# samuel-vitorino/lm.rs

Measured on AMD Instinct MI355X. Metric: decode tok/s + %HBM-roofline, Llama-3.2-1B Q8_0 @1/2/4/8 MI355X vs CPU ref, higher is better.
Workload: dtype int8xint8->int32, f32 combine; 1 GPU; llama-3.2-1b Q8_0 (gs=128) greedy decode, 5-token synthetic prompt then 3164 tokens, batch 1; parallelism=single GPU, image_bytes=1274634496

## Files before the change

lm.rs_amd/csrc/lmrs_kernels.hip:

```cpp
#include <hip/hip_ext.h>
#include <mutex>
#include <map>
#include <set>
#include <tuple>
#include <utility>

#include "lmrs_device_math.h"
#include "lmrs_kernels.h"
#include "lmrs_stage.h"

namespace lmrs {

constexpr int kBlock = 256;


constexpr int kMaxP = 16;

template <int NP>
__device__ __forceinline__ void rmsnorm_inplace(float4 (&v)[NP], const float4 (&wv)[NP], int n, float eps,
                                                int add_unit, float* scratch) {
    const int t = threadIdx.x;
    const int P = (n + 1023) >> 10;
    const int JP = (n >> 3) + 4;
#pragma unroll
// ... 49 lines not shown
            if (e < n) {
                float4 o;
                if (add_unit) {
                    o.x = (1.0f + wv[i].x) * (ss * v[i].x); o.y = (1.0f + wv[i].y) * (ss * v[i].y);
                    o.z = (1.0f + wv[i].z) * (ss * v[i].z); o.w = (1.0f + wv[i].w) * (ss * v[i].w);
                } else {
                    o.x = wv[i].x * (ss * v[i].x); o.y = wv[i].y * (ss * v[i].y);
                    o.z = wv[i].z * (ss * v[i].z); o.w = wv[i].w * (ss * v[i].w);
                }
                v[i] = o;
            }
        }
    }
}

template <bool Q4, int NP>
__device__ __forceinline__ void quantize_to_lds(const float4 (&v)[NP], int n, int8_t* xq, float* xs, void* gq, float* gs_out) {
    const int t = threadIdx.x;
    const int P = (n + 1023) >> 10;
#pragma unroll
    for (int i = 0; i < NP; ++i) {
        if (i < P) {
            const int e = i * 1024 + t * 4;
            const bool live = e < n;
            float m = 0.0f;
            if (live) m = fmaxf(fmaxf(fabsf(v[i].x), fabsf(v[i].y)), fmaxf(fabsf(v[i].z), fabsf(v[i].w)));
            m = group32_max(m);
            if (live) {
                if constexpr (!Q4) {
                    const float scale = m / 127.0f, inv = __builtin_amdgcn_rcpf(scale);
                    float dev = 0.0f;
                    int q0 = quant_q8_try(v[i].x, inv, dev), q1 = quant_q8_try(v[i].y, inv, dev);
                    int q2 = quant_q8_try(v[i].z, inv, dev), q3 = quant_q8_try(v[i].w, inv, dev);
                    if (quant_slow(m, dev)) { q0 = quant_q8(v[i].x, scale); q1 = quant_q8(v[i].y, scale); q2 = quant_q8(v[i].z, scale); q3 = quant_q8(v[i].w, scale); }
                    const unsigned packed = (q0 & 0xff) | ((q1 & 0xff) << 8) | ((q2 & 0xff) << 16) | ((unsigned)(q3 & 0xff) << 24);
                    *reinterpret_cast<unsigned*>(xq + e) = packed;
                    if ((t & 31) == 0) xs[e >> 7] = scale;
                    if (gq) {
                        *reinterpret_cast<unsigned*>(reinterpret_cast<int8_t*>(gq) + e) = packed;
                        if ((t & 31) == 0) gs_out[e >> 7] = scale;
                    }
                } else {
                    const float scale = m / -8.0f;
                    const unsigned a = quant_q4(v[i].x, scale), b = quant_q4(v[i].y, scale);
                    const unsigned c = quant_q4(v[i].z, scale), d = quant_q4(v[i].w, scale);
                    const int base = e & ~7, k0 = e & 7;
                    xq[base + (k0 >> 1) + 0] = (int8_t)((int)a - 8);
                    xq[base + 4 + (k0 >> 1) + 0] = (int8_t)((int)b - 8);
                    xq[base + (k0 >> 1) + 1] = (int8_t)((int)c - 8);
                    xq[base + 4 + (k0 >> 1) + 1] = (int8_t)((int)d - 8);
                    if ((t & 31) == 0) xs[e >> 7] = scale;
                    if (gq) {
                        uint8_t* g8 = reinterpret_cast<uint8_t*>(gq);
                        g8[(e >> 1) + 0] = (uint8_t)(a | (b << 4));
                        g8[(e >> 1) + 1] = (uint8_t)(c | (d << 4));
                        if ((t & 31) == 0) gs_out[e >> 7] = scale;
                    }
                }
            }
        }
    }
}

template <int NP>
__device__ __forceinline__ void load_vec(float4 (&v)[NP], const float* __restrict__ x, int n) {
    const int t = threadIdx.x;
    const int P = (n + 1023) >> 10;
#pragma unroll
    for (int i = 0; i < NP; ++i) {
        if (i < P) {
            const int e = i * 1024 + t * 4;
            if (e < n) v[i] = *reinterpret_cast<const float4*>(x + e);
        }
    }
}

struct TailPre { int pos, prompt_end; uint32_t tok_next; };
__device__ __forceinline__ TailPre tail_preload(const ArgmaxArgs& a) {
    TailPre p; p.pos = a.st->pos; p.prompt_end = a.st->prompt_end; p.tok_next = a.tokens[p.pos + 1]; return p;
}
__device__ __forceinline__ void argmax_tail(const ArgmaxArgs& a, float best, int best_i, int nan0, const TailPre& pre) {
    __shared__ float sv[kBlock / 64];
    __shared__ int si[kBlock / 64];
    __shared__ uint32_t s_next;
    if (threadIdx.x == 0 && a.tail_row > 0 && (0.0f > best || (0.0f == best && a.tail_row < best_i))) { best = 0.0f; best_i = a.tail_row; }
#pragma unroll
    for (int off = 32; off >= 1; off >>= 1) {
        const float ov = __shfl_xor(best, off); const int oi = __shfl_xor(best_i, off);
        if (ov > best || (ov == best && oi < best_i)) { best = ov; best_i = oi; }
    }
    if ((threadIdx.x & 63) == 0) { sv[threadIdx.x >> 6] = best; si[threadIdx.x >> 6] = best_i; }
    nan0 = __syncthreads_or(nan0);
    if (threadIdx.x == 0) {
        for (int w = 1; w < kBlock / 64; ++w)
            if (sv[w] > best || (sv[w] == best && si[w] < best_i)) { best = sv[w]; best_i = si[w]; }
        int win = best_i;
        if (nan0 || win == 0x7fffffff) win = 0;
        const int pos = pre.pos;
        uint32_t next = (uint32_t)win;
        if (pos + 1 >= pre.prompt_end) a.tokens[pos + 1] = next;
        else next = pre.tok_next;
        a.st->pos = pos + 1;
        a.st->step_count += 1;
        if (a.seq) *a.seq += 1u;
        s_next = next;
    }
    __syncthreads();
    const uint32_t token = s_next;
    if (a.emb.q4 == 0 && a.emb.dim > 0 && (a.emb.dim & 7) == 0 && a.emb.dim <= 8 * 4 * kBlock) {
        const int8_t* qrow = reinterpret_cast<const int8_t*>(a.emb.emb_q) + (size_t)token * a.emb.dim;
        const float* srow = a.emb.emb_s + ((size_t)token * a.emb.dim) / kGS;
        uint2 q8[4]; float sc[4];
#pragma unroll
        for (int k = 0; k < 4; ++k) {
            const int e = (k * kBlock + (int)threadIdx.x) * 8;
            const bool live = e < a.emb.dim;
            q8[k] = *reinterpret_cast<const uint2*>(qrow + (live ? e : 0));
            sc[k] = srow[(live ? e : 0) / kGS];
        }
#pragma unroll
        for (int k = 0; k < 4; ++k) {
            const int e = (k * kBlock + (int)threadIdx.x) * 8;
            if (e < a.emb.dim) {
                float o[8];
#pragma unroll
                for (int u = 0; u < 8; ++u) {
                    const int b = (int)(int8_t)(((u < 4 ? q8[k].x : q8[k].y) >> (8 * (u & 3))) & 0xff);
                    float v = (float)b * sc[k];
                    if (a.emb.do_scale) v = v * a.emb.scale;
                    o[u] = v;
                }
                *reinterpret_cast<float4*>(a.emb.x + e) = make_float4(o[0], o[1], o[2], o[3]);
                *reinterpret_cast<float4*>(a.emb.x + e + 4) = make_float4(o[4], o[5], o[6], o[7]);
            }
        }
    } else if (a.emb.q4 == 1 && a.emb.dim > 0 && (a.emb.dim & 7) == 0 && a.emb.dim <= 8 * 4 * kBlock) {
        const uint8_t* qrow = reinterpret_cast<const uint8_t*>(a.emb.emb_q) + ((size_t)token * a.emb.dim) / 2;
        const float* srow = a.emb.emb_s + ((size_t)token * a.emb.dim) / kGS;
        unsigned q4w[4]; float sc[4];
#pragma unroll
        for (int k = 0; k < 4; ++k) {
            const int e = (k * kBlock + (int)threadIdx.x) * 8;
            const bool live = e < a.emb.dim;
            q4w[k] = *reinterpret_cast<const unsigned*>(qrow + (live ? e : 0) / 2);
            sc[k] = srow[(live ? e : 0) / kGS];
        }
#pragma unroll
        for (int k = 0; k < 4; ++k) {
            const int e = (k * kBlock + (int)threadIdx.x) * 8;
            if (e < a.emb.dim) {
                float o[8];
#pragma unroll
                for (int u = 0; u < 8; ++u) {
                    const int nib = (int)((q4w[k] >> (4 * u)) & 0xfu) - 8;
                    float v = (float)nib * sc[k];
                    if (a.emb.do_scale) v = v * a.emb.scale;
                    o[u] = v;
                }
                *reinterpret_cast<float4*>(a.emb.x + e) = make_float4(o[0], o[1], o[2], o[3]);
                *reinterpret_cast<float4*>(a.emb.x + e + 4) = make_float4(o[4], o[5], o[6], o[7]);
            }
        }
    } else {
        for (int i = threadIdx.x; i < a.emb.dim; i += kBlock) {
            float v = dequant_elem(a.emb.emb_q, a.emb.emb_s, a.emb.q4, (size_t)token * a.emb.dim + i);
            if (a.emb.do_scale) v = v * a.emb.scale;
            a.emb.x[i] = v;
        }
    }
}

__device__ __forceinline__ unsigned cls_tag(const GemvArgs& a) { return (*a.tail.cls_seq + 1u) & 0x7ffu; }
__device__ __forceinline__ void cls_publish(const GemvArgs& a, int bid, unsigned tag, float best, int best_i) {
    const unsigned hi = best_i < 0 ? (0x80000000u | (tag << 20)) : ((tag << 20) | (best_i == 0x7fffffff ? 0xfffffu : (unsigned)best_i));
    __hip_atomic_store(a.tail.part_pk + bid, ((unsigned long long)hi << 32) | __float_as_uint(best), __ATOMIC_RELAXED, __HIP_MEMORY_SCOPE_AGENT);
}
__device__ __forceinline__ void cls_consumer(const GemvArgs& a, int nprod, const TailPre& pre, unsigned tag) {
    if (a.dbg && threadIdx.x == 0) a.dbg[4] = wall_clock64();
    float bv; int bi, nan0;
    for (unsigned spins = 0;; ++spins) {
        bv = __uint_as_float(0xff800000u); bi = 0x7fffffff; nan0 = 0;
        int ok = 1;
        for (int i = threadIdx.x; i < nprod; i += kBlock) {
            const unsigned long long pk = __hip_atomic_load(a.tail.part_pk + i, __ATOMIC_RELAXED, __HIP_MEMORY_SCOPE_AGENT);
            const unsigned hi = (unsigned)(pk >> 32);
            if (((hi >> 20) & 0x7ffu) != tag) { ok = 0; continue; }
            if (hi & 0x80000000u) { nan0 = 1; continue; }
            const float v = __uint_as_float((unsigned)pk); const int idx = (hi & 0xfffffu) == 0xfffffu ? 0x7fffffff : (int)(hi & 0xfffffu);
            if (v > bv || (v == bv && idx < bi)) { bv = v; bi = idx; }
        }
        if (__syncthreads_and(ok)) break;
// ... 701 lines not shown
                const int i = i0 + u;
                if constexpr (kBlock % HS4 == 0) { row[u] = r0 + i * (kBlock / HS4); col[u] = c4; }
                else { const int f = (int)threadIdx.x + i * kBlock; row[u] = f / HS4; col[u] = f - row[u] * HS4; }
                if constexpr (SCALE) sc[u] = rowscale[row[u] < nrows ? row[u] : nrows - 1];
            }
#pragma unroll
            for (int u = 0; u < 4; ++u) {
                const int i = i0 + u;
                if (i < NF && (AttGeom<HS>::ALIGNED || row[u] < nrows)) {
                    float4 v = rg[i];
                    if constexpr (SCALE) { v.x = sc[u] * v.x; v.y = sc[u] * v.y; v.z = sc[u] * v.z; v.w = sc[u] * v.w; }
                    *reinterpret_cast<float4*>(tile + row[u] * RS + col[u] * 4) = v;
                }
            }
        }
    }
    if (patch_t >= t0 && patch_t < t0 + ct) {
        const int fb = (patch_t - t0) * HS4, d = ((int)threadIdx.x - fb) & (kBlock - 1);
        if (d < HS4) {
            float4 v = *reinterpret_cast<const float4*>(patch + d * 4);
            if constexpr (SCALE) { const float ap = rowscale[patch_t - t0]; v.x = ap * v.x; v.y = ap * v.y; v.z = ap * v.z; v.w = ap * v.w; }
            *reinterpret_cast<float4*>(tile + (patch_t - t0) * RS + d * 4) = v;
        }
    }
}

#define ATT_STAMP(k) do { if (a.dbg && threadIdx.x == 0 && blockIdx.x == 0) a.dbg[k] = wall_clock64(); } while (0)

struct AttPre { float q0, q1, k0, k1; float2 cs; };

typedef float f32x4v __attribute__((ext_vector_type(4)));
__device__ __forceinline__ float* att_k_head(const AttnArgs& a, int kvh, int hs) {
    return a.k_cache + ((size_t)a.layer * a.n_kv_heads + kvh) * hs * (size_t)a.seq_len;
}
template <int NG>
__device__ __forceinline__ void att_kload(f32x4v (&dst)[NG], __amdgpu_buffer_rsrc_t krs, int voff, int g0, int S) {
#pragma unroll
    for (int u = 0; u < NG; ++u) {
        const auto t = __builtin_amdgcn_raw_buffer_load_b128(krs, voff, (g0 + u) * S * 16, 0);
        dst[u] = f32x4v{__uint_as_float(t[0]), __uint_as_float(t[1]), __uint_as_float(t[2]), __uint_as_float(t[3])};
    }
}
template <int NG>
__device__ __forceinline__ float att_kuse(float score, const f32x4v (&src)[NG], const float4* q4, int g0) {
#pragma unroll
    for (int u = 0; u < NG; ++u) {
        const float4 qq = q4[g0 + u];
        float pr;
        pr = qq.x * src[u].x; score = score + pr;
        pr = qq.y * src[u].y; score = score + pr;
        pr = qq.z * src[u].z; score = score + pr;
        pr = qq.w * src[u].w; score = score + pr;
    }
    return score;
}
template <int HS, int NG>
__device__ __forceinline__ float att_score_chain(f32x4v (&kk)[NG], __amdgpu_buffer_rsrc_t krs, int voff, const float* q, int S) {
    constexpr int HS4 = HS / 4;
    f32x4v kb[NG];
    float score = 0.0f;
    const float4* q4 = reinterpret_cast<const float4*>(q);
#pragma unroll
    for (int g0 = 0; g0 < HS4; g0 += 2 * NG) {
        if (g0 + NG < HS4) att_kload<NG>(kb, krs, voff, g0 + NG, S);
        score = att_kuse<NG>(score, kk, q4, g0);
        asm volatile("" : "+v"(score) : : "memory");
        if (g0 + NG < HS4) {
            if (g0 + 2 * NG < HS4) att_kload<NG>(kk, krs, voff, g0 + 2 * NG, S);
            score = att_kuse<NG>(score, kb, q4, g0 + NG);
            asm volatile("" : "+v"(score) : : "memory");
        }
    }
    return score;
}

__device__ __forceinline__ float2 rope_rotate(float v0, float v1, float fcr, float fci) {
    const float a0 = v0 * fcr, a1 = v1 * fci, b0 = v0 * fci, b1 = v1 * fcr;
    return make_float2(a0 - a1, b0 + b1);
}
__device__ __forceinline__ void k_store_pair(float* k, int S, int pos, int j, int half, float r0, float r1) {
    k[(((size_t)(j >> 2) * S + pos) << 2) + (j & 3)] = r0;
    k[(((size_t)((j + half) >> 2) * S + pos) << 2) + ((j + half) & 3)] = r1;
}
__device__ __forceinline__ float gemma_cap_window(float score, int wpos, int t) {
    score = score / 50.0f;
    score = (float)tanh((double)score);
    score = score * 50.0f;
    return score + (((unsigned)(wpos - t) <= 4096u) ? 0.0f : -2.3819763e38f);
}
template <int HS4>
__device__ __forceinline__ float tile_score(const float4* k, int ks, const float* qs) {
    constexpr int GB = 4;
    static_assert(HS4 % (2 * GB) == 0, "head size");
    const float4* q4 = reinterpret_cast<const float4*>(qs);
    auto dot = [](float score, const float4 (&q)[GB], const float4 (&kk)[GB]) __attribute__((always_inline)) {
#pragma unroll
        for (int u = 0; u < GB; ++u) {
            float pr;
            pr = q[u].x * kk[u].x; score = score + pr;
            pr = q[u].y * kk[u].y; score = score + pr;
            pr = q[u].z * kk[u].z; score = score + pr;
            pr = q[u].w * kk[u].w; score = score + pr;
        }
        return score;
    };
    float score = 0.0f;
    float4 ka[GB], qa[GB], kb[GB], qb[GB];
#pragma unroll
    for (int u = 0; u < GB; ++u) { ka[u] = k[u * ks]; qa[u] = q4[u]; }
#pragma unroll
    for (int g0 = 0; g0 < HS4; g0 += 2 * GB) {
#pragma unroll
        for (int u = 0; u < GB; ++u) { kb[u] = k[(g0 + GB + u) * ks]; qb[u] = q4[g0 + GB + u]; }
        asm volatile("" : "+v"(score) : : "memory");
        score = dot(score, qa, ka);
        if (g0 + 2 * GB < HS4) {
#pragma unroll
            for (int u = 0; u < GB; ++u) { ka[u] = k[(g0 + 2 * GB + u) * ks]; qa[u] = q4[g0 + 2 * GB + u]; }
        }
        asm volatile("" : "+v"(score) : : "memory");
        score = dot(score, qb, kb);
    }
    return score;
}
struct AttTag { const unsigned long long* gran; unsigned tag; int att_dim, kv_dim; int* err; };
template <int NG>
__device__ __forceinline__ void poll_granules(const unsigned long long* const (&gp)[NG], const AttTag& tg, int layer, unsigned long long (&xg)[NG]) {
    auto sweep = [&](unsigned long long (&x)[NG]) __attribute__((always_inline)) {
#pragma unroll
        for (int k = 0; k < NG; ++k) x[k] = __hip_atomic_load(gp[k], __ATOMIC_RELAXED, __HIP_MEMORY_SCOPE_AGENT);
    };
    auto fresh = [&](const unsigned long long (&x)[NG]) __attribute__((always_inline)) {
        bool ok = true;
#pragma unroll
        for (int k = 0; k < NG; ++k) ok = ok && (unsigned)(x[k] >> 32) == tg.tag;
        return __all(ok) != 0;
    };
    auto take = [&](const unsigned long long (&x)[NG]) __attribute__((always_inline)) {
#pragma unroll
        for (int k = 0; k < NG; ++k) xg[k] = x[k];
    };
    unsigned long long xa[NG], xb[NG];
    sweep(xa);
    for (unsigned spins = 0;; ++spins) {
        sweep(xb);
        if (fresh(xa)) { take(xa); break; }
        sweep(xa);
        if (fresh(xb)) { take(xb); break; }
        if (spins > kTagSpinMax || (spins & 1023) == 1023) {
            const int e = __hip_atomic_load(tg.err, __ATOMIC_RELAXED, __HIP_MEMORY_SCOPE_AGENT);
            if (e != 0 || spins > kTagSpinMax) {
                if (e == 0) __hip_atomic_store(tg.err, layer + 1, __ATOMIC_RELAXED, __HIP_MEMORY_SCOPE_AGENT);
                take(xb);
                break;
            }
        }
    }
}
__device__ __forceinline__ void granules_of(const AttTag& tg, int h, int kvh, int hs, int d, const unsigned long long** gp) {
    gp[0] = tg.gran + h * hs + d; gp[1] = tg.gran + tg.att_dim + kvh * hs + d; gp[2] = tg.gran + tg.att_dim + tg.kv_dim + kvh * hs + d;
}

template <int HS, int NF, bool COH, bool PRE = false, bool GEMMA = false, bool ROT = false, bool TAG = false>
__device__ __forceinline__ void attention_body(const AttnArgs& a, int h, int pos, char* smem, uint64_t etab, const AttPre& pre = AttPre(), const AttTag& tg = AttTag()) {
    static_assert(!PRE || HS / 2 <= kBlock, "one RoPE pair per lane");
    static_assert(!TAG || (HS <= kBlock && !COH && !PRE && !ROT), "granule polling: one value of each vector per lane");
// ... 259 lines not shown
        }
    }
    if (a.dbg && lane == 0 && blockIdx.x == 0) a.dbg[3] = wall_clock64();

    int wpos = pos;
    if constexpr (GEMMA) { const int wb = a.st->win_base; wpos = wb >= 0 ? wb : pos; }
    const float sqrt_hs = sqrtf((float)HS), ninf = __uint_as_float(0xff800000u);
    float sc[NPASS];
    float lmax = ninf;
#pragma unroll
    for (int p = 0; p < NPASS; ++p) {
        sc[p] = ninf;
        if (64 * p < T) {
            const int t = 64 * p + lane;
            float score = tile_score<HS4>(kt + t, TW, qs) / sqrt_hs;
            if constexpr (GEMMA) score = gemma_cap_window(score, wpos, t);
            sc[p] = t < T ? score : ninf;
            lmax = fmaxf(lmax, sc[p]);
        }
    }
    if (a.dbg && lane == 0 && blockIdx.x == 0) a.dbg[4] = wall_clock64();
    const float mx = wave64_max(lmax);
    float ex[NPASS];
#pragma unroll
    for (int p = 0; p < NPASS; ++p) {
        ex[p] = 0.0f;
        if (64 * p < T) {
            const int t = 64 * p + lane;
            const float e = expf_glibc_t(t < T ? sc[p] - mx : 0.0f, etab);
            ex[p] = t < T ? e : 0.0f;
        }
    }
    float sum = 0.0f;
#pragma unroll
    for (int p = 0; p < NPASS; ++p) {
        if (64 * p < T) {
            const int left = T - 64 * p;
            sum = wave_serial_sum(sum, ex[p], left >= 64 ? 4 : (left + 15) >> 4);
        }
    }
    float ap_lane = 0.0f;
#pragma unroll
    for (int p = 0; p < NPASS; ++p) {
        if (64 * p < T) {
            const int t = 64 * p + lane;
            const float w = ex[p] / sum;
            att[t] = t < pos ? w : 0.0f;
            if ((pos >> 6) == p) ap_lane = w;
        }
    }
    const float a_pos = __builtin_bit_cast(float, __builtin_amdgcn_readlane(__builtin_bit_cast(int, ap_lane), pos & 63));
    if (a.dbg && lane == 0 && blockIdx.x == 0) a.dbg[5] = wall_clock64();
    float o[ND];
#pragma unroll
    for (int i = 0; i < ND; ++i) o[i] = 0.0f;
#pragma unroll
    for (int t0 = 0; t0 < TW; t0 += 16) {
        if (t0 < pos) {
            float4 w4[4];
#pragma unroll
            for (int u = 0; u < 4; ++u) w4[u] = reinterpret_cast<const float4*>(att)[t0 / 4 + u];
#pragma unroll
            for (int u = 0; u < 4; ++u)
#pragma unroll
                for (int i = 0; i < ND; ++i) {
                    float pr;
                    pr = w4[u].x * v[i][t0 + 4 * u + 0]; o[i] = o[i] + pr;
                    pr = w4[u].y * v[i][t0 + 4 * u + 1]; o[i] = o[i] + pr;
                    pr = w4[u].z * v[i][t0 + 4 * u + 2]; o[i] = o[i] + pr;
                    pr = w4[u].w * v[i][t0 + 4 * u + 3]; o[i] = o[i] + pr;
                }
        }
    }
#pragma unroll
    for (int i = 0; i < ND; ++i) {
        const int d = lane + 64 * i;
        const float pr = a_pos * vnew[i];
        o[i] = o[i] + pr;
        if (d < HS) a.out[h * HS + d] = o[i];
    }
    if (a.dbg && lane == 0 && blockIdx.x == 0) a.dbg[7] = wall_clock64();
}

constexpr size_t kPairSmem = (size_t)(2 * 2 * 64 + 128 + 16 + 16) * 4 + (size_t)16 * 128 * 16 + (size_t)64 * 64 * 4;
template <bool GEMMA>
__device__ __forceinline__ void attention_pair_tag(const AttnArgs& a, const int h, const int pos, char* smem, const uint64_t etab, const AttTag& tg) {
    constexpr int HS = 64, HS4 = 16, TW = 128, half = 32;
    const int lane = threadIdx.x & 63, wv = __builtin_amdgcn_readfirstlane((int)threadIdx.x >> 6);
    const bool two = pos >= 64;
    if (wv > (two ? 1 : 0)) return;
    const int tb = two ? 64 * wv : 0;
    const int kv_mul = a.n_heads / a.n_kv_heads, kvh = h / kv_mul, kv_dim = a.n_kv_heads * HS;
    const int T = pos + 1, S = a.seq_len;
    float* base = reinterpret_cast<float*>(smem);
    float* qs = base + wv * 2 * HS;
    float* kn = qs + HS;
    float* att = base + 4 * HS;
    float* red = att + TW + 16;
    float4* kt = reinterpret_cast<float4*>(red + 16);
    float* prod = reinterpret_cast<float*>(kt + HS4 * TW);
    float* kT = att_k_head(a, kvh, HS);
    const float* vbase = a.v_cache + (size_t)a.layer * S * kv_dim + kvh * HS;
    if (a.dbg && lane == 0 && wv == 0 && blockIdx.x == 0) a.dbg[0] = wall_clock64();

    const float2 cs = *reinterpret_cast<const float2*>(a.rope + ((size_t)pos * half + (lane < half ? lane : 0)) * 2);
    if (tb < pos) {
#pragma unroll
        for (int g = 0; g < HS4; ++g)
            __builtin_amdgcn_global_load_lds((const LMRS_GLOBAL void*)(kT + ((size_t)g * S + tb + lane) * 4),
                                             (__attribute__((address_space(3))) void*)(kt + g * TW + tb), 16, 0, 0);
    }
    float v[64];
    const __amdgpu_buffer_rsrc_t vrs = __builtin_amdgcn_make_buffer_rsrc(const_cast<float*>(vbase), 0, 0x7fffffff, 0x00020000);
    const int vrow = kv_dim * 4, vb0 = tb * vrow;
    auto vblock = [&](auto self, auto u0c) __attribute__((always_inline)) -> void {
        constexpr int u0 = decltype(u0c)::value;
        if constexpr (u0 < 64) {
            if (tb + u0 < pos) {
#pragma unroll
                for (int u = 0; u < 16; ++u) v[u0 + u] = __uint_as_float(__builtin_amdgcn_raw_buffer_load_b32(vrs, lane * 4, vb0 + (u0 + u) * vrow, 0));
                self(self, std::integral_constant<int, u0 + 16>());
            }
        }
    };
    vblock(vblock, std::integral_constant<int, 0>());
#pragma unroll
    for (int u = 0; u < 64; ++u) { v[u] = tb + u < pos ? v[u] : 0.0f; asm volatile("" : "+v"(v[u])); }
    if (a.dbg && lane == 0 && wv == 0 && blockIdx.x == 0) a.dbg[1] = wall_clock64();

    unsigned long long xg[3];
    {
        const unsigned long long* gp[3];
        granules_of(tg, h, kvh, HS, lane, gp);
        poll_granules<3>(gp, tg, a.layer, xg);
    }
    asm volatile("s_waitcnt vmcnt(0)" ::: "memory");
    if (a.dbg && lane == 0 && wv == 0 && blockIdx.x == 0) a.dbg[2] = wall_clock64();
    const float vnew = __uint_as_float((unsigned)xg[2]);
    qs[lane] = __uint_as_float((unsigned)xg[0]); kn[lane] = __uint_as_float((unsigned)xg[1]);
    if (lane < half) {
        const int j = lane;
        const float2 rq = rope_rotate(qs[j], qs[j + half], cs.x, cs.y);
        qs[j] = rq.x; qs[j + half] = rq.y;
        const float2 rk = rope_rotate(kn[j], kn[j + half], cs.x, cs.y);
        if (wv == 0) k_store_pair(kT, S, pos, j, half, rk.x, rk.y);
        if ((pos >> 6) == (two ? wv : 0)) k_store_pair(reinterpret_cast<float*>(kt), TW, pos, j, half, rk.x, rk.y);
    }
    if (a.dbg && lane == 0 && wv == 0 && blockIdx.x == 0) a.dbg[3] = wall_clock64();

    int wpos = pos;
    if constexpr (GEMMA) { const int wb = a.st->win_base; wpos = wb >= 0 ? wb : pos; }
    const float sqrt_hs = sqrtf((float)HS), ninf = __uint_as_float(0xff800000u);
    const int t = tb + lane;
    float sc;
    {
        float score = tile_score<HS4>(kt + t, TW, qs) / sqrt_hs;
        if constexpr (GEMMA) score = gemma_cap_window(score, wpos, t);
        sc = t < T ? score : ninf;
    }
    if (a.dbg && lane == 0 && wv == 0 && blockIdx.x == 0) a.dbg[4] = wall_clock64();
    float mx = wave64_max(sc);
    if (two) {
        if (lane == 0) red[wv] = mx;
        lds_barrier();
        mx = fmaxf(red[0], red[1]);
    }
    const float e0 = expf_glibc_t(t < T ? sc - mx : 0.0f, etab);
    const float ex = t < T ? e0 : 0.0f;
    float sum;
    if (!two) {
        sum = wave_serial_sum(0.0f, ex, (T + 15) >> 4);
    } else {
        if (wv == 0) { sum = wave_serial_sum(0.0f, ex, 4); if (lane == 0) red[2] = sum; }
        lds_barrier();
        if (wv == 1) { sum = wave_serial_sum(red[2], ex, (T - 64 + 15) >> 4); if (lane == 0) red[3] = sum; }
        lds_barrier();
        sum = red[3];
    }
    const float w = ex / sum;
    att[t] = t < pos ? w : 0.0f;
    const bool own_pos = (pos >> 6) == (two ? wv : 0);
    float a_pos = 0.0f;
    if (own_pos) a_pos = __builtin_bit_cast(float, __builtin_amdgcn_readlane(__builtin_bit_cast(int, w), pos & 63));
    if (a.dbg && lane == 0 && wv == 0 && blockIdx.x == 0) a.dbg[5] = wall_clock64();
    if (two && wv == 1) {
        if (lane == 0) red[4] = a_pos;
#pragma unroll
        for (int u0 = 0; u0 < 64; u0 += 16) {
            if (64 + u0 < pos) {
                float4 w4[4];
#pragma unroll
                for (int u = 0; u < 4; ++u) w4[u] = reinterpret_cast<const float4*>(att)[(64 + u0) / 4 + u];
#pragma unroll
                for (int u = 0; u < 4; ++u) {
                    prod[(u0 + 4 * u + 0) * HS + lane] = w4[u].x * v[u0 + 4 * u + 0];
                    prod[(u0 + 4 * u + 1) * HS + lane] = w4[u].y * v[u0 + 4 * u + 1];
                    prod[(u0 + 4 * u + 2) * HS + lane] = w4[u].z * v[u0 + 4 * u + 2];
                    prod[(u0 + 4 * u + 3) * HS + lane] = w4[u].w * v[u0 + 4 * u + 3];
                }
            }
        }
        lds_barrier();
        return;
    }
    float o = 0.0f;
#pragma unroll
    for (int u0 = 0; u0 < 64; u0 += 16) {
        if (u0 < pos) {
            float4 w4[4];
#pragma unroll
            for (int u = 0; u < 4; ++u) w4[u] = reinterpret_cast<const float4*>(att)[u0 / 4 + u];
#pragma unroll
            for (int u = 0; u < 4; ++u) {
                float pr;
                pr = w4[u].x * v[u0 + 4 * u + 0]; o = o + pr;
                pr = w4[u].y * v[u0 + 4 * u + 1]; o = o + pr;
                pr = w4[u].z * v[u0 + 4 * u + 2]; o = o + pr;
                pr = w4[u].w * v[u0 + 4 * u + 3]; o = o + pr;
            }
        }
    }
    if (two) {
        lds_barrier();
        a_pos = red[4];
#pragma unroll
        for (int u0 = 0; u0 < 64; u0 += 16) {
            if (64 + u0 < pos) {
                float pb[16];
#pragma unroll
                for (int u = 0; u < 16; ++u) pb[u] = prod[(u0 + u) * HS + lane];
#pragma unroll
                for (int u = 0; u < 16; ++u) o = o + pb[u];
            }
        }
    }
    {
        const float pr = a_pos * vnew;
        o = o + pr;
        a.out[h * HS + lane] = o;
    }
    if (a.dbg && lane == 0 && wv == 0 && blockIdx.x == 0) a.dbg[7] = wall_clock64();
}

constexpr int kMultiWaves = 4;
constexpr size_t kMultiSmem = (size_t)(kMultiWaves * 2 * 64 + 64 * kMultiWaves + 16 + 32) * 4 + (size_t)(kMultiWaves - 1) * 64 * 64 * 4;
template <bool GEMMA>
__device__ __forceinline__ void attention_multi_tag(const AttnArgs& a, const int h, const int pos, char* smem, const uint64_t etab, const AttTag& tg) {
    constexpr int HS = 64, HS4 = 16, half = 32;
    const int lane = threadIdx.x & 63, wv = __builtin_amdgcn_readfirstlane((int)threadIdx.x >> 6);
    const int nw = (pos >> 6) + 1 < kMultiWaves ? (pos >> 6) + 1 : kMultiWaves;
    if (wv >= nw) return;
    const int tb = 64 * wv, t = tb + lane;
    const int kv_mul = a.n_heads / a.n_kv_heads, kvh = h / kv_mul, kv_dim = a.n_kv_heads * HS;
    const int T = pos + 1, S = a.seq_len;
    float* base = reinterpret_cast<float*>(smem);
    float* qs = base + wv * 2 * HS;
    float* kn = qs + HS;
    float* att = base + kMultiWaves * 2 * HS;
    float* red = att + 64 * kMultiWaves + 16;
    float* prod = red + 32;
    float* kT = att_k_head(a, kvh, HS);
    const float* vbase = a.v_cache + (size_t)a.layer * S * kv_dim + kvh * HS;
    if (a.dbg && lane == 0 && wv == 0 && blockIdx.x == 0) a.dbg[0] = wall_clock64();

    const float2 cs = *reinterpret_cast<const float2*>(a.rope + ((size_t)pos * half + (lane < half ? lane : 0)) * 2);
    f32x4v kreg[HS4];
    {
        const int tk = t < S ? t : S - 1;
        if (tb < pos) {
#pragma unroll
            for (int g = 0; g < HS4; ++g) kreg[g] = *reinterpret_cast<const f32x4v*>(kT + ((size_t)g * S + tk) * 4);
        } else {
#pragma unroll
            for (int g = 0; g < HS4; ++g) kreg[g] = f32x4v{0.0f, 0.0f, 0.0f, 0.0f};
        }
    }
    float v[64];
    const __amdgpu_buffer_rsrc_t vrs = __builtin_amdgcn_make_buffer_rsrc(const_cast<float*>(vbase), 0, 0x7fffffff, 0x00020000);
    const int vrow = kv_dim * 4;
    auto vblock = [&](auto self, auto u0c) __attribute__((always_inline)) -> void {
        constexpr int u0 = decltype(u0c)::value;
        if constexpr (u0 < 64) {
            if (tb + u0 < pos) {
#pragma unroll
                for (int u = 0; u < 16; ++u) {
                    const int row = tb + u0 + u < S ? tb + u0 + u : S - 1;
                    v[u0 + u] = __uint_as_float(__builtin_amdgcn_raw_buffer_load_b32(vrs, lane * 4, row * vrow, 0));
                }
                self(self, std::integral_constant<int, u0 + 16>());
            }
        }
    };
    vblock(vblock, std::integral_constant<int, 0>());
#pragma unroll
    for (int u = 0; u < 64; ++u) { v[u] = tb + u < pos ? v[u] : 0.0f; asm volatile("" : "+v"(v[u])); }
    if (a.dbg && lane == 0 && wv == 0 && blockIdx.x == 0) a.dbg[1] = wall_clock64();

    unsigned long long xg[3];
    {
        const unsigned long long* gp[3];
        granules_of(tg, h, kvh, HS, lane, gp);
        poll_granules<3>(gp, tg, a.layer, xg);
    }
    asm volatile("s_waitcnt vmcnt(0)" ::: "memory");
    if (a.dbg && lane == 0 && wv == 0 && blockIdx.x == 0) a.dbg[2] = wall_clock64();
    const float vnew = __uint_as_float((unsigned)xg[2]);
    qs[lane] = __uint_as_float((unsigned)xg[0]); kn[lane] = __uint_as_float((unsigned)xg[1]);
    const bool own_pos = (pos >> 6) == wv;
    if (lane < half) {
        const int j = lane;
        const float2 rq = rope_rotate(qs[j], qs[j + half], cs.x, cs.y);
        qs[j] = rq.x; qs[j + half] = rq.y;
        const float2 rk = rope_rotate(kn[j], kn[j + half], cs.x, cs.y);
        kn[j] = rk.x; kn[j + half] = rk.y;
        if (wv == 0) k_store_pair(kT, S, pos, j, half, rk.x, rk.y);
    }
    if (own_pos) {
#pragma unroll
        for (int g = 0; g < HS4; ++g) {
            const float4 n4 = reinterpret_cast<const float4*>(kn)[g];
            const bool me = lane == (pos & 63);
            kreg[g][0] = me ? n4.x : kreg[g][0]; kreg[g][1] = me ? n4.y : kreg[g][1]; kreg[g][2] = me ? n4.z : kreg[g][2]; kreg[g][3] = me ? n4.w : kreg[g][3];
        }
    }
    if (a.dbg && lane == 0 && wv == 0 && blockIdx.x == 0) a.dbg[3] = wall_clock64();

    int wpos = pos;
    if constexpr (GEMMA) { const int wb = a.st->win_base; wpos = wb >= 0 ? wb : pos; }
    const float sqrt_hs = sqrtf((float)HS), ninf = __uint_as_float(0xff800000u);
    float sc;
    {
        float score = 0.0f;
#pragma unroll
        for (int g = 0; g < HS4; ++g) {
            const float4 q4 = reinterpret_cast<const float4*>(qs)[g];
            float pr;
            pr = q4.x * kreg[g][0]; score = score + pr;
            pr = q4.y * kreg[g][1]; score = score + pr;
            pr = q4.z * kreg[g][2]; score = score + pr;
            pr = q4.w * kreg[g][3]; score = score + pr;
        }
        score = score / sqrt_hs;
        if constexpr (GEMMA) score = gemma_cap_window(score, wpos, t);
        sc = t < T ? score : ninf;
    }
    if (a.dbg && lane == 0 && wv == 0 && blockIdx.x == 0) a.dbg[4] = wall_clock64();
    float mx = wave64_max(sc);
    if (nw > 1) {
        if (lane == 0) red[wv] = mx;
        lds_barrier();
        mx = red[0];
        for (int w = 1; w < nw; ++w) mx = fmaxf(mx, red[w]);
    }
    const float e0 = expf_glibc_t(t < T ? sc - mx : 0.0f, etab);
    const float ex = t < T ? e0 : 0.0f;
    float sum;
    if (nw == 1) {
        sum = wave_serial_sum(0.0f, ex, (T + 15) >> 4);
    } else {
        for (int s = 0; s < nw; ++s) {
            if (wv == s) {
                const int left = T - 64 * s;
                const float part = wave_serial_sum(s ? red[8 + s - 1] : 0.0f, ex, left >= 64 ? 4 : (left + 15) >> 4);
                if (lane == 0) red[8 + s] = part;
            }
            lds_barrier();
        }
        sum = red[8 + nw - 1];
    }
    const float w = ex / sum;
    att[t] = t < pos ? w : 0.0f;
    float a_pos = 0.0f;
    if (own_pos) a_pos = __builtin_bit_cast(float, __builtin_amdgcn_readlane(__builtin_bit_cast(int, w), pos & 63));
    if (a.dbg && lane == 0 && wv == 0 && blockIdx.x == 0) a.dbg[5] = wall_clock64();
    if (wv > 0) {
        if (own_pos && lane == 0) red[4] = a_pos;
        float* mine = prod + (size_t)(wv - 1) * 64 * HS;
#pragma unroll
        for (int u0 = 0; u0 < 64; u0 += 16) {
            if (tb + u0 < pos) {
                float4 w4[4];
#pragma unroll
                for (int u = 0; u < 4; ++u) w4[u] = reinterpret_cast<const float4*>(att)[(tb + u0) / 4 + u];
#pragma unroll
                for (int u = 0; u < 4; ++u) {
                    mine[(u0 + 4 * u + 0) * HS + lane] = w4[u].x * v[u0 + 4 * u + 0];
                    mine[(u0 + 4 * u + 1) * HS + lane] = w4[u].y * v[u0 + 4 * u + 1];
                    mine[(u0 + 4 * u + 2) * HS + lane] = w4[u].z * v[u0 + 4 * u + 2];
                    mine[(u0 + 4 * u + 3) * HS + lane] = w4[u].w * v[u0 + 4 * u + 3];
                }
            }
        }
        lds_barrier();
        return;
    }
    float o = 0.0f;
#pragma unroll
    for (int u0 = 0; u0 < 64; u0 += 16) {
        if (u0 < pos) {
            float4 w4[4];
#pragma unroll
            for (int u = 0; u < 4; ++u) w4[u] = reinterpret_cast<const float4*>(att)[u0 / 4 + u];
#pragma unroll
            for (int u = 0; u < 4; ++u) {
                float pr;
                pr = w4[u].x * v[u0 + 4 * u + 0]; o = o + pr;
                pr = w4[u].y * v[u0 + 4 * u + 1]; o = o + pr;
                pr = w4[u].z * v[u0 + 4 * u + 2]; o = o + pr;
                pr = w4[u].w * v[u0 + 4 * u + 3]; o = o + pr;
            }
        }
    }
    if (nw > 1) {
        lds_barrier();
        a_pos = red[4];
        for (int k0 = 0; k0 < 64 * (kMultiWaves - 1); k0 += 16) {
            if (64 + k0 < pos) {
                float pb[16];
#pragma unroll
                for (int u = 0; u < 16; ++u) pb[u] = prod[(k0 + u) * HS + lane];
#pragma unroll
                for (int u = 0; u < 16; ++u) o = o + pb[u];
            }
        }
    }
    {
        const float pr = a_pos * vnew;
        o = o + pr;
        a.out[h * HS + lane] = o;
    }
    if (a.dbg && lane == 0 && wv == 0 && blockIdx.x == 0) a.dbg[7] = wall_clock64();
}

template <int HS> struct QuadGeom {
    static constexpr int HS4 = HS / 4, ND = (HS + 63) / 64, NH2 = (HS / 2 + 63) / 64;
    static constexpr int KPW = HS <= 128 ? 32 : 16, TWK = 4 * KPW;
    static constexpr int NPASS = TWK / 64;
    static constexpr size_t SMEM = (size_t)(4 * 2 * HS + TWK + 16 + 32) * 4 + (size_t)HS4 * TWK * 16;
    static_assert((size_t)3 * KPW * ND * 64 * 4 <= (size_t)HS4 * TWK * 16, "the products alias the K tile");
};
template <int HS, bool GEMMA>
__device__ __forceinline__ void attention_quad_tag(const AttnArgs& a, const int h, const int pos, char* smem, const uint64_t etab, const AttTag& tg) {
    using Q = QuadGeom<HS>;
    constexpr int HS4 = Q::HS4, ND = Q::ND, NH2 = Q::NH2, KPW = Q::KPW, TWK = Q::TWK, half = HS / 2;
    const int lane = threadIdx.x & 63, wv = __builtin_amdgcn_readfirstlane((int)threadIdx.x >> 6);
    const int kpw = (KPW == 32 && pos >= 64) ? 32 : 16;
    const int tb = kpw * wv;
    const int kv_mul = a.n_heads / a.n_kv_heads, kvh = h / kv_mul, kv_dim = a.n_kv_heads * HS;
    const int T = pos + 1, S = a.seq_len;
    float* base = reinterpret_cast<float*>(smem);
    float* qs = base + wv * 2 * HS;
    float* kn = qs + HS;
    float* att = base + 4 * 2 * HS;
    float* red = att + TWK + 16;
    float4* kt = reinterpret_cast<float4*>(red + 32);
    float* prod = reinterpret_cast<float*>(kt);
    float* kT = att_k_head(a, kvh, HS);
    const float* vbase = a.v_cache + (size_t)a.layer * S * kv_dim + kvh * HS;
    if (a.dbg && lane == 0 && wv == 0 && blockIdx.x == 0) a.dbg[0] = wall_clock64();

    float2 cs[NH2];
#pragma unroll
    for (int i = 0; i < NH2; ++i) { const int j = lane + 64 * i; cs[i] = *reinterpret_cast<const float2*>(a.rope + ((size_t)pos * half + (j < half ? j : 0)) * 2); }
#pragma unroll
    for (int p = 0; p < Q::NPASS; ++p) {
        if (64 * p < pos) {
#pragma unroll
            for (int gg = 0; gg < HS4 / 4; ++gg) {
                const int g = wv * (HS4 / 4) + gg;
                __builtin_amdgcn_global_load_lds((const LMRS_GLOBAL void*)(kT + ((size_t)g * S + 64 * p + lane) * 4),
                                                 (__attribute__((address_space(3))) void*)(kt + g * TWK + 64 * p), 16, 0, 0);
            }
        }
    }
    float v[ND][KPW];
    const __amdgpu_buffer_rsrc_t vrs = __builtin_amdgcn_make_buffer_rsrc(const_cast<float*>(vbase), 0, 0x7fffffff, 0x00020000);
    const int vrow = kv_dim * 4, vb0 = tb * vrow;
    auto vblock = [&](auto self, auto u0c) __attribute__((always_inline)) -> void {
        constexpr int u0 = decltype(u0c)::value;
        if constexpr (u0 < KPW) {
            if (u0 < kpw && tb + u0 < pos) {
#pragma unroll
                for (int u = 0; u < 16; ++u)
#pragma unroll
                    for (int i = 0; i < ND; ++i) {
                        const int d = lane + 64 * i;
                        v[i][u0 + u] = __uint_as_float(__builtin_amdgcn_raw_buffer_load_b32(vrs, (d < HS ? d : 0) * 4, vb0 + (u0 + u) * vrow, 0));
                    }
                self(self, std::integral_constant<int, u0 + 16>());
            }
        }
    };
    vblock(vblock, std::integral_constant<int, 0>());
#pragma unroll
    for (int u = 0; u < KPW; ++u)
#pragma unroll
        for (int i = 0; i < ND; ++i) { v[i][u] = (u < kpw && tb + u < pos) ? v[i][u] : 0.0f; asm volatile("" : "+v"(v[i][u])); }
    if (a.dbg && lane == 0 && wv == 0 && blockIdx.x == 0) a.dbg[1] = wall_clock64();

    unsigned long long xg[3 * ND];
    {
        const unsigned long long* gp[3 * ND];
#pragma unroll
        for (int i = 0; i < ND; ++i) { const int d = lane + 64 * i; granules_of(tg, h, kvh, HS, d < HS ? d : 0, gp + 3 * i); }
        poll_granules<3 * ND>(gp, tg, a.layer, xg);
    }
    asm volatile("s_waitcnt vmcnt(0)" ::: "memory");
// ... 1164 lines not shown
```

Before: 1391 tok/s.

## Cut barriers in argmax tail and small-context attention via lane swaps and padded LDS

The argmax tail now has every thread redo the cross-wave reduction itself, which removes a shared-variable broadcast and one block barrier. In the pair and multi-wave attention paths, RoPE partners come from a permlane32 swap rather than an LDS round trip. The softmax sum is built by publishing exps once and having every wave run the serial sum redundantly, replacing the chain of one barrier per wave. The partial products move to a per-lane padded layout written as float4 and read back by a new chain_rows16 helper. This adds LDS space and redundant per-thread work, and chain_rows16 is only forward-declared in the shown code.

```diff
diff --git a/lm.rs_amd/csrc/lmrs_kernels.hip b/lm.rs_amd/csrc/lmrs_kernels.hip
--- a/lm.rs_amd/csrc/lmrs_kernels.hip
+++ b/lm.rs_amd/csrc/lmrs_kernels.hip
@@ -155,7 +155,6 @@
 __device__ __forceinline__ void argmax_tail(const ArgmaxArgs& a, float best, int best_i, int nan0, const TailPre& pre) {
     __shared__ float sv[kBlock / 64];
     __shared__ int si[kBlock / 64];
-    __shared__ uint32_t s_next;
     if (threadIdx.x == 0 && a.tail_row > 0 && (0.0f > best || (0.0f == best && a.tail_row < best_i))) { best = 0.0f; best_i = a.tail_row; }
 #pragma unroll
     for (int off = 32; off >= 1; off >>= 1) {
@@ -164,22 +163,21 @@
     }
     if ((threadIdx.x & 63) == 0) { sv[threadIdx.x >> 6] = best; si[threadIdx.x >> 6] = best_i; }
     nan0 = __syncthreads_or(nan0);
+    best = sv[0]; best_i = si[0];
+#pragma unroll
+    for (int w = 1; w < kBlock / 64; ++w)
+        if (sv[w] > best || (sv[w] == best && si[w] < best_i)) { best = sv[w]; best_i = si[w]; }
+    int win = best_i;
+    if (nan0 || win == 0x7fffffff) win = 0;
+    const int pos = pre.pos;
+    const bool feed = pos + 1 >= pre.prompt_end;
+    const uint32_t token = feed ? (uint32_t)win : pre.tok_next;
     if (threadIdx.x == 0) {
-        for (int w = 1; w < kBlock / 64; ++w)
-            if (sv[w] > best || (sv[w] == best && si[w] < best_i)) { best = sv[w]; best_i = si[w]; }
-        int win = best_i;
-        if (nan0 || win == 0x7fffffff) win = 0;
-        const int pos = pre.pos;
-        uint32_t next = (uint32_t)win;
-        if (pos + 1 >= pre.prompt_end) a.tokens[pos + 1] = next;
-        else next = pre.tok_next;
+        if (feed) a.tokens[pos + 1] = token;
         a.st->pos = pos + 1;
         a.st->step_count += 1;
         if (a.seq) *a.seq += 1u;
-        s_next = next;
-    }
-    __syncthreads();
-    const uint32_t token = s_next;
+    }
     if (a.emb.q4 == 0 && a.emb.dim > 0 && (a.emb.dim & 7) == 0 && a.emb.dim <= 8 * 4 * kBlock) {
         const int8_t* qrow = reinterpret_cast<const int8_t*>(a.emb.emb_q) + (size_t)token * a.emb.dim;
         const float* srow = a.emb.emb_s + ((size_t)token * a.emb.dim) / kGS;
@@ -1047,6 +1045,13 @@
     k[(((size_t)(j >> 2) * S + pos) << 2) + (j & 3)] = r0;
     k[(((size_t)((j + half) >> 2) * S + pos) << 2) + ((j + half) & 3)] = r1;
 }
+__device__ __forceinline__ float lane_plus32(float v) {
+    const auto sw = __builtin_amdgcn_permlane32_swap(__float_as_uint(v), __float_as_uint(v), false, false);
+    return __uint_as_float(sw[1]);
+}
+constexpr int prod_pitch(int keys) { return keys + 4; }
+constexpr int kProdPad = 48;
+__device__ __forceinline__ float chain_rows16(float o, const float4* row, int nb);
 __device__ __forceinline__ float gemma_cap_window(float score, int wpos, int t) {
     score = score / 50.0f;
     score = (float)tanh((double)score);
@@ -1472,10 +1477,10 @@
     if (a.dbg && lane == 0 && blockIdx.x == 0) a.dbg[7] = wall_clock64();
 }
 
-constexpr size_t kPairSmem = (size_t)(2 * 2 * 64 + 128 + 16 + 16) * 4 + (size_t)16 * 128 * 16 + (size_t)64 * 64 * 4;
+constexpr size_t kPairSmem = (size_t)(2 * 64 + 128 + 128 + 16 + 16) * 4 + (size_t)16 * 128 * 16 + (size_t)(64 * prod_pitch(64) + kProdPad) * 4;
 template <bool GEMMA>
 __device__ __forceinline__ void attention_pair_tag(const AttnArgs& a, const int h, const int pos, char* smem, const uint64_t etab, const AttTag& tg) {
-    constexpr int HS = 64, HS4 = 16, TW = 128, half = 32;
+    constexpr int HS = 64, HS4 = 16, TW = 128, half = 32, PP = prod_pitch(64);
     const int lane = threadIdx.x & 63, wv = __builtin_amdgcn_readfirstlane((int)threadIdx.x >> 6);
     const bool two = pos >= 64;
     if (wv > (two ? 1 : 0)) return;
@@ -1483,8 +1488,8 @@
     const int kv_mul = a.n_heads / a.n_kv_heads, kvh = h / kv_mul, kv_dim = a.n_kv_heads * HS;
     const int T = pos + 1, S = a.seq_len;
     float* base = reinterpret_cast<float*>(smem);
-    float* qs = base + wv * 2 * HS;
-    float* kn = qs + HS;
+    float* qs = base + wv * HS;
+    float* exs = base + 2 * HS;
     float* att = base + 4 * HS;
     float* red = att + TW + 16;
     float4* kt = reinterpret_cast<float4*>(red + 16);
@@ -1527,14 +1532,17 @@
     asm volatile("s_waitcnt vmcnt(0)" ::: "memory");
     if (a.dbg && lane == 0 && wv == 0 && blockIdx.x == 0) a.dbg[2] = wall_clock64();
     const float vnew = __uint_as_float((unsigned)xg[2]);
-    qs[lane] = __uint_as_float((unsigned)xg[0]); kn[lane] = __uint_as_float((unsigned)xg[1]);
-    if (lane < half) {
-        const int j = lane;
-        const float2 rq = rope_rotate(qs[j], qs[j + half], cs.x, cs.y);
-        qs[j] = rq.x; qs[j + half] = rq.y;
-        const float2 rk = rope_rotate(kn[j], kn[j + half], cs.x, cs.y);
-        if (wv == 0) k_store_pair(kT, S, pos, j, half, rk.x, rk.y);
-        if ((pos >> 6) == (two ? wv : 0)) k_store_pair(reinterpret_cast<float*>(kt), TW, pos, j, half, rk.x, rk.y);
+    {
+        const float q0 = __uint_as_float((unsigned)xg[0]), k0 = __uint_as_float((unsigned)xg[1]);
+        const float q1 = lane_plus32(q0), k1 = lane_plus32(k0);
+        if (lane < half) {
+            const int j = lane;
+            const float2 rq = rope_rotate(q0, q1, cs.x, cs.y);
+            qs[j] = rq.x; qs[j + half] = rq.y;
+            const float2 rk = rope_rotate(k0, k1, cs.x, cs.y);
+            if (wv == 0) k_store_pair(kT, S, pos, j, half, rk.x, rk.y);
+            if ((pos >> 6) == (two ? wv : 0)) k_store_pair(reinterpret_cast<float*>(kt), TW, pos, j, half, rk.x, rk.y);
+        }
     }
     if (a.dbg && lane == 0 && wv == 0 && blockIdx.x == 0) a.dbg[3] = wall_clock64();
 
@@ -1561,11 +1569,11 @@
     if (!two) {
         sum = wave_serial_sum(0.0f, ex, (T + 15) >> 4);
     } else {
-        if (wv == 0) { sum = wave_serial_sum(0.0f, ex, 4); if (lane == 0) red[2] = sum; }
+        exs[t] = ex;
         lds_barrier();
-        if (wv == 1) { sum = wave_serial_sum(red[2], ex, (T - 64 + 15) >> 4); if (lane == 0) red[3] = sum; }
-        lds_barrier();
-        sum = red[3];
+        const float eo = exs[(tb ^ 64) + lane];
+        sum = wave_serial_sum(0.0f, wv == 0 ? ex : eo, 4);
+        sum = wave_serial_sum(sum, wv == 0 ? eo : ex, (T - 64 + 15) >> 4);
     }
     const float w = ex / sum;
     att[t] = t < pos ? w : 0.0f;
@@ -1581,13 +1589,11 @@
                 float4 w4[4];
 #pragma unroll
                 for (int u = 0; u < 4; ++u) w4[u] = reinterpret_cast<const float4*>(att)[(64 + u0) / 4 + u];
-#pragma unroll
-                for (int u = 0; u < 4; ++u) {
-                    prod[(u0 + 4 * u + 0) * HS + lane] = w4[u].x * v[u0 + 4 * u + 0];
-                    prod[(u0 + 4 * u + 1) * HS + lane] = w4[u].y * v[u0 + 4 * u + 1];
-                    prod[(u0 + 4 * u + 2) * HS + lane] = w4[u].z * v[u0 + 4 * u + 2];
-                    prod[(u0 + 4 * u + 3) * HS + lane] = w4[u].w * v[u0 + 4 * u + 3];
-                }
+                asm volatile("" ::: "memory");
+#pragma unroll
+                for (int u = 0; u < 4; ++u)
+                    *reinterpret_cast<float4*>(prod + lane * PP + u0 + 4 * u) =
+                        make_float4(w4[u].x * v[u0 + 4 * u + 0], w4[u].y * v[u0 + 4 * u + 1], w4[u].z * v[u0 + 4 * u + 2], w4[u].w * v[u0 + 4 * u + 3]);
             }
         }
         lds_barrier();
@@ -1613,16 +1619,7 @@
     if (two) {
         lds_barrier();
         a_pos = red[4];
-#pragma unroll
-        for (int u0 = 0; u0 < 64; u0 += 16) {
-            if (64 + u0 < pos) {
-                float pb[16];
-#pragma unroll
-                for (int u = 0; u < 16; ++u) pb[u] = prod[(u0 + u) * HS + lane];
-#pragma unroll
-                for (int u = 0; u < 16; ++u) o = o + pb[u];
-            }
-        }
+        o = chain_rows16(o, reinterpret_cast<const float4*>(prod + lane * PP), (pos - 64 + 15) >> 4);
     }
     {
         const float pr = a_pos * vnew;
@@ -1633,10 +1630,10 @@
 }
 
 constexpr int kMultiWaves = 4;
-constexpr size_t kMultiSmem = (size_t)(kMultiWaves * 2 * 64 + 64 * kMultiWaves + 16 + 32) * 4 + (size_t)(kMultiWaves - 1) * 64 * 64 * 4;
+constexpr size_t kMultiSmem = (size_t)(kMultiWaves * 2 * 64 + 2 * 64 * kMultiWaves + 16 + 32) * 4 + (size_t)(64 * prod_pitch((kMultiWaves - 1) * 64) + kProdPad) * 4;
 template <bool GEMMA>
 __device__ __forceinline__ void attention_multi_tag(const AttnArgs& a, const int h, const int pos, char* smem, const uint64_t etab, const AttTag& tg) {
-    constexpr int HS = 64, HS4 = 16, half = 32;
+    constexpr int HS = 64, HS4 = 16, half = 32, PP = prod_pitch((kMultiWaves - 1) * 64);
     const int lane = threadIdx.x & 63, wv = __builtin_amdgcn_readfirstlane((int)threadIdx.x >> 6);
     const int nw = (pos >> 6) + 1 < kMultiWaves ? (pos >> 6) + 1 : kMultiWaves;
     if (wv >= nw) return;
@@ -1647,7 +1644,8 @@
     float* qs = base + wv * 2 * HS;
     float* kn = qs + HS;
     float* att = base + kMultiWaves * 2 * HS;
-    float* red = att + 64 * kMultiWaves + 16;
+    float* exs = att + 64 * kMultiWaves + 16;
+    float* red = exs + 64 * kMultiWaves;
     float* prod = red + 32;
     float* kT = att_k_head(a, kvh, HS);
     const float* vbase = a.v_cache + (size_t)a.layer * S * kv_dim + kvh * HS;
@@ -1695,15 +1693,18 @@
     asm volatile("s_waitcnt vmcnt(0)" ::: "memory");
     if (a.dbg && lane == 0 && wv == 0 && blockIdx.x == 0) a.dbg[2] = wall_clock64();
     const float vnew = __uint_as_float((unsigned)xg[2]);
-    qs[lane] = __uint_as_float((unsigned)xg[0]); kn[lane] = __uint_as_float((unsigned)xg[1]);
     const bool own_pos = (pos >> 6) == wv;
-    if (lane < half) {
-        const int j = lane;
-        const float2 rq = rope_rotate(qs[j], qs[j + half], cs.x, cs.y);
-        qs[j] = rq.x; qs[j + half] = rq.y;
-        const float2 rk = rope_rotate(kn[j], kn[j + half], cs.x, cs.y);
-        kn[j] = rk.x; kn[j + half] = rk.y;
-        if (wv == 0) k_store_pair(kT, S, pos, j, half, rk.x, rk.y);
+    {
+        const float q0 = __uint_as_float((unsigned)xg[0]), k0 = __uint_as_float((unsigned)xg[1]);
+        const float q1 = lane_plus32(q0), k1 = lane_plus32(k0);
+        if (lane < half) {
+            const int j = lane;
+            const float2 rq = rope_rotate(q0, q1, cs.x, cs.y);
+            qs[j] = rq.x; qs[j + half] = rq.y;
+            const float2 rk = rope_rotate(k0, k1, cs.x, cs.y);
+            kn[j] = rk.x; kn[j + half] = rk.y;
+            if (wv == 0) k_store_pair(kT, S, pos, j, half, rk.x, rk.y);
+        }
     }
     if (own_pos) {
 #pragma unroll
@@ -1748,15 +1749,19 @@
     if (nw == 1) {
         sum = wave_serial_sum(0.0f, ex, (T + 15) >> 4);
     } else {
-        for (int s = 0; s < nw; ++s) {
-            if (wv == s) {
+        exs[t] = ex;
+        lds_barrier();
+        float eo[kMultiWaves];
+#pragma unroll
+        for (int s = 0; s < kMultiWaves; ++s) eo[s] = s < nw ? exs[64 * s + lane] : 0.0f;
+        sum = 0.0f;
+#pragma unroll
+        for (int s = 0; s < kMultiWaves; ++s) {
+            if (s < nw) {
                 const int left = T - 64 * s;
-                const float part = wave_serial_sum(s ? red[8 + s - 1] : 0.0f, ex, left >= 64 ? 4 : (left + 15) >> 4);
-                if (lane == 0) red[8 + s] = part;
-            }
-            lds_barrier();
-        }
-        sum = red[8 + nw - 1];
+                sum = wave_serial_sum(sum, s == wv ? ex : eo[s], left >= 64 ? 4 : (left + 15) >> 4);
+            }
+        }
     }
     const float w = ex / sum;
     att[t] = t < pos ? w : 0.0f;
@@ -1765,7 +1770,7 @@
     if (a.dbg && lane == 0 && wv == 0 && blockIdx.x == 0) a.dbg[5] = wall_clock64();
     if (wv > 0) {
         if (own_pos && lane == 0) red[4] = a_pos;
-        float* mine = prod + (size_t)(wv - 1) * 64 * HS;
+        float* mine = prod + lane * PP + (wv - 1) * 64;
 #pragma unroll
         for (int u0 = 0; u0 < 64; u0 += 16) {
             if (tb + u0 < pos) {
@@ -1773,12 +1778,9 @@
 #pragma unroll
                 for (int u = 0; u < 4; ++u) w4[u] = reinterpret_cast<const float4*>(att)[(tb + u0) / 4 + u];
 #pragma unroll
-                for (int u = 0; u < 4; ++u) {
-                    mine[(u0 + 4 * u + 0) * HS + lane] = w4[u].x * v[u0 + 4 * u + 0];
-                    mine[(u0 + 4 * u + 1) * HS + lane] = w4[u].y * v[u0 + 4 * u + 1];
-                    mine[(u0 + 4 * u + 2) * HS + lane] = w4[u].z * v[u0 + 4 * u + 2];
-                    mine[(u0 + 4 * u + 3) * HS + lane] = w4[u].w * v[u0 + 4 * u + 3];
-                }
+                for (int u = 0; u < 4; ++u)
+                    *reinterpret_cast<float4*>(mine + u0 + 4 * u) =
+                        make_float4(w4[u].x * v[u0 + 4 * u + 0], w4[u].y * v[u0 + 4 * u + 1], w4[u].z * v[u0 + 4 * u + 2], w4[u].w * v[u0 + 4 * u + 3]);
             }
         }
         lds_barrier();
@@ -1804,15 +1806,7 @@
     if (nw > 1) {
         lds_barrier();
         a_pos = red[4];
-        for (int k0 = 0; k0 < 64 * (kMultiWaves - 1); k0 += 16) {
-            if (64 + k0 < pos) {
-                float pb[16];
-#pragma unroll
-                for (int u = 0; u < 16; ++u) pb[u] = prod[(k0 + u) * HS + lane];
-#pragma unroll
-                for (int u = 0; u < 16; ++u) o = o + pb[u];
-            }
-        }
+        o = chain_rows16(o, reinterpret_cast<const float4*>(prod + lane * PP), (pos - 64 + 15) >> 4);
     }
     {
         const float pr = a_pos * vnew;
```

After: 1391 tok/s (median of 2 runs). Within noise of the previous version (-0.0%).
